# xin-fight/Research-and-Implementation-of-Image-Dehazing-Algorithm-Based-on-Vision-Transformer

Hardware: AMD Instinct MI355X
Metric: train patches/sec (128x128, embed_dim=32) (higher is better)
Workload: dtype f32; 1 GPU; Uformer_ProbSparse train step E=32 ps=128 per-GPU bs=32 fp32 Charbonnier+CR(VGG19, seeded-random weights) + AdamW (BASELINE configs[1]); global_batch=32, parallelism=dp1, arithmetic=fp32 storage/accumulate; products 6xbf16 MFMA, dropped <= 2^-24, split_terms=6

## Files before the change

### include/dehaze_hip.h

```cpp
#ifndef DEHAZE_HIP_H
#define DEHAZE_HIP_H

#include <stdint.h>

#ifdef __cplusplus
extern "C" {
#endif

#define DHZ_OK 0
#define DHZ_EINVAL (-22)
#define DHZ_ELAUNCH (-5)

#define DHZ_F32 0
#define DHZ_BF16 1

#define DHZ_NTOK 64
#define DHZ_NTOP 25

int dhz_abi_version(void);
const char* dhz_last_error(void);
const char* dhz_build_id(void);
int dhz_set_reserved_cus(int k);
int dhz_get_reserved_cus(void);
int dhz_grid_cus(void);
// ... 83 lines not shown
                        const float* bd, const float* b2, const float* drop_scale, float* out, float* xn_save, float* stats_save,
                        float* u_save, float* tp_save, float* z_save, int B, int Hres, int Wres, int C, void* stream);
int dhz_leff_prepack6(const float* w1, const float* w2, void* w6, int C, void* stream);

int dhz_linear_fwd(const float* x, int ldx, const float* w, const float* bias, float* y, int ldy, int T, int N, int K,
                   void* stream);
int dhz_linear_dgrad(const float* dy, int ldy, const float* w, float* dx, int ldx, int T, int N, int K, void* stream);
int dhz_linear_tile(int rows, int out_features);

int dhz_linear_fwd_split(const float* x, int ldx, const float* w, const float* bias, float* y, int ldy, int T, int N, int K,
                         int terms, void* stream);
int dhz_linear_dgrad_split(const float* dy, int ldy, const float* w, float* dx, int ldx, int T, int N, int K, int terms,
                           void* stream);
int dhz_linear_fwd_split6(const float* x, int ldx, const void* w_hi, const void* w_mid, const void* w_lo, const float* bias, float* y,
                          int ldy, int T, int N, int K, void* stream);
int dhz_linear_dgrad_split6(const float* dy, int ldy, const void* w_hi, const void* w_mid, const void* w_lo, float* dx, int ldx, int T,
                            int N, int K, void* stream);
int dhz_linear_fwd_split6_res(const float* x, int ldx, const void* w_hi, const void* w_mid, const void* w_lo, const float* bias,
                              const float* res, const float* scale, float* out, int ldo, int T, int N, int K, int tokens_per_image,
                              int Hres, int Wres, int shift, int windowed, void* stream);
int dhz_linear_split6_tile(int mode, int T, int N, int K);
int dhz_linear_fwd_split_res(const float* x, int ldx, const float* w, const float* bias, const float* res, const float* scale, float* out,
                             int ldo, int T, int N, int K, int tokens_per_image, int Hres, int Wres, int shift, int windowed, int terms,
                             void* stream);
int dhz_linear_dgrad_split_scaled(const float* dy, int ldy, const float* w, const float* scale, float* dx, int ldx, int T, int N, int K,
                                  int tokens_per_image, int terms, void* stream);
int dhz_linear_fwd_bf16_res(const void* x, int ldx, const void* w, const float* bias, const void* res, const float* scale, void* out, int ldo,
                            int T, int N, int K, int tokens_per_image, int Hres, int Wres, int shift, int windowed, void* stream);
int dhz_split3_planes(const float* src, int64_t n, void* hi, void* mid, void* lo, void* stream);
int dhz_split3_planes_t(const float* src, void* hi, void* mid, void* lo, const int* desc, int nmat, int ntiles, void* stream);
int dhz_bf16_transpose_batched(const float* src, void* dst, const int* desc, int nmat, int ntiles, void* stream);
int dhz_linear_wgrad_split(const float* dy, int ldy, const float* x, int ldx, int T, int nmat, int nper, int K, float* const* dw,
                           float* const* db, const float* row_scale, int rows_per_scale, int terms, void* stream);

int dhz_linear_fwd_bf16(const void* x, int ldx, const void* w, const float* bias, void* y, int ldy, int T, int N, int K,
                        void* stream);
int dhz_linear_dgrad_bf16(const void* dy, int ldy, const void* w, void* dx, int ldx, int T, int N, int K, void* stream);
int dhz_linear_wgrad_bf16(const void* dy, int ldy, const void* x, int ldx, int T, int nmat, int nper, int K,
                          float* const* dw, float* const* db, void* stream);

int dhz_gelu_fwd_dt(const void* u, void* y, int64_t n, int dtype, void* stream);
int dhz_gelu_bwd_dt(const void* dy, const void* u, void* du, int64_t n, const float* scale, int64_t elems_per_scale, int dtype, void* stream);
int dhz_ln_partition_fwd_dt(const void* x, const float* gamma, const float* beta, void* xw, float* stats, int B, int Hres,
                            int Wres, int C, int shift, int partition, int dtype, void* stream);
int dhz_ln_partition_bwd_dt(const void* dxw, const void* x, const float* gamma, const float* stats, const void* dres, void* dx,
                            float* dgamma, float* dbeta, int B, int Hres, int Wres, int C, int shift, int partition, int dtype,
                            void* stream);
int dhz_ln_partition_bwd_lay(const void* dxw, const void* x, const float* gamma, const float* stats, const void* dres, void* dx,
                             float* dgamma, float* dbeta, int B, int Hres, int Wres, int C, int shift, int partition, int dres_windowed,
                             int dx_windowed, int dx_shift, int dtype, void* stream);
int dhz_ln_partition_bwd_lay2(const void* dxw, const void* x, const float* gamma, const float* stats, const void* dres, void* dx,
                              float* dgamma, float* dbeta, int B, int Hres, int Wres, int C, int shift, int partition, int dres_windowed,
                              int dx_windowed, int dx_shift, void* dx2, const float* scale2, int dtype, void* stream);
int dhz_reverse_residual_fwd_dt(const void* yw, const void* shortcut, const float* scale, void* out, int B, int Hres, int Wres,
                                int C, int shift, int partition, int dtype, void* stream);
int dhz_reverse_residual_bwd_dt(const void* dout, const float* scale, void* dyw, int B, int Hres, int Wres, int C, int shift,
                                int partition, int dtype, void* stream);
int dhz_leff_dwconv_fwd_dt(const void* u, const float* w, const float* b, void* t, void* z, int B, int Hres, int Wres, int Ch,
                           int dtype, void* stream);
int dhz_leff_dwconv_bwd_dt(const void* dz, const void* u, const void* t, const float* w, void* du, float* dw, float* db, int B,
                           int Hres, int Wres, int Ch, int dtype, void* stream);
int dhz_leff_dwconv_bwd_scaled_dt(const void* dz, const void* u, const void* t, const float* w, void* du, float* dw, float* db,
                                  const float* dz_scale, int B, int Hres, int Wres, int Ch, int dtype, void* stream);
int dhz_leff_dwconv_bwd_dy(const float* dy, int ldy, const void* w2t_hi, const void* w2t_mid, const void* w2t_lo, const float* u,
                           const float* tpre, const float* wd, float* du, float* dw, float* db, const float* dz_scale, int B, int Hres,
                           int Wres, int C, int Ch, void* stream);
// ... 169 lines not shown
```

### research-and-implementation-of-image-dehazing-algorithm-based-on-vision-transformer_amd/dehaze_hip/_lib.py

```python
import ctypes
import os

_HERE = os.path.dirname(os.path.abspath(__file__))
LIB_PATH = os.environ.get("DHZ_LIB_PATH") or os.path.join(_HERE, "libdehaze_hip.so")

c_f = ctypes.c_void_p
c_p = ctypes.c_void_p
c_i = ctypes.c_int
c_l = ctypes.c_int64
c_fl = ctypes.c_float

SIGNATURES = {
    "dhz_abi_version": [],
    "dhz_last_error": [],
    "dhz_build_id": [],
    "dhz_set_reserved_cus": [ctypes.c_int],
    "dhz_gelu_fwd_dt": [ctypes.c_void_p, ctypes.c_void_p, ctypes.c_int64, ctypes.c_int, ctypes.c_void_p],
    "dhz_gelu_bwd_dt": [ctypes.c_void_p, ctypes.c_void_p, ctypes.c_void_p, ctypes.c_int64, ctypes.c_void_p, ctypes.c_int64, ctypes.c_int, ctypes.c_void_p],
    "dhz_get_reserved_cus": [],
    "dhz_set_deterministic": [ctypes.c_int],
    "dhz_get_deterministic": [],
    "dhz_set_det_workspace": [ctypes.c_void_p, ctypes.c_size_t],
    "dhz_grid_cus": [],
    "dhz_ps_attn_fwd": [c_f, c_f, c_f, c_i, c_p, c_f, c_f, c_f, c_i, c_p, c_i, c_i, c_i, c_i, c_p],
# ... 35 lines not shown
    "dhz_winograd43_conv3x3_pool": [c_f, c_f, c_f, c_f, c_f, c_i, c_i, c_i, c_i, c_i, c_p],
    "dhz_winograd_conv3x3_slices": [c_f, c_f, c_f, c_i, c_f, c_f, c_f, c_f, c_i, c_i, c_i, c_i, c_i, c_i, c_p],
    "dhz_winograd43_conv3x3_slices": [c_f, c_f, c_f, c_i, c_f, c_f, c_f, c_f, c_i, c_i, c_i, c_i, c_i, c_i, c_p],
    "dhz_winograd_slices": [c_i, c_i, c_i, c_i, c_i],
    "dhz_maxpool2x2_blocked_fwd": [c_f, c_f, c_i, c_i, c_i, c_p],
    "dhz_maxpool2x2_blocked_bwd": [c_f, c_f, c_f, c_i, c_i, c_i, c_p],
    "dhz_layout_blocked8": [c_f, c_f, c_i, c_i, c_i, c_i, c_f, c_i, c_p],
    "dhz_leff_fused_fwd": [c_f] * 16 + [c_i, c_i, c_i, c_i, c_p],
    "dhz_leff_fused_fwd6": [c_f] * 15 + [c_i, c_i, c_i, c_i, c_p],
    "dhz_leff_prepack6": [c_f, c_f, c_p, c_i, c_p],
    "dhz_linear_fwd": [c_f, c_i, c_f, c_f, c_f, c_i, c_i, c_i, c_i, c_p],
    "dhz_linear_dgrad": [c_f, c_i, c_f, c_f, c_i, c_i, c_i, c_i, c_p],
    "dhz_input_proj_fwd": [c_f, c_f, c_f, c_f, c_i, c_i, c_i, c_i, c_fl, c_p],
    "dhz_input_proj_bwd": [c_f, c_f, c_f, c_f, c_f, c_i, c_i, c_i, c_i, c_fl, c_p],
    "dhz_conv4s2_fwd": [c_f, c_f, c_f, c_f, c_i, c_i, c_i, c_i, c_i, c_p],
    "dhz_conv4s2_dgrad": [c_f, c_f, c_f, c_i, c_i, c_i, c_i, c_i, c_p],
    "dhz_conv4s2_wgrad": [c_f, c_f, c_f, c_f, c_i, c_i, c_i, c_i, c_i, c_p],
    "dhz_input_proj_fwd_dt": [c_f, c_f, c_f, c_f, c_i, c_i, c_i, c_i, c_fl, c_i, c_p],
    "dhz_input_proj_bwd_dt": [c_f, c_f, c_f, c_f, c_f, c_i, c_i, c_i, c_i, c_fl, c_i, c_p],
    "dhz_thin_conv3x3_fwd_dt": [c_f, c_f, c_f, c_f, c_i, c_i, c_i, c_i, c_i, c_p],
    "dhz_thin_conv3x3_dgrad_dt": [c_f, c_f, c_f, c_i, c_i, c_i, c_i, c_i, c_p],
    "dhz_thin_conv3x3_wgrad_dt": [c_f, c_f, c_f, c_f, c_i, c_i, c_i, c_i, c_i, c_p],
    "dhz_vgg_prepack_bf16": [c_f, c_f, c_i, c_i, c_i, c_p],
    "dhz_vgg_conv3x3_bf16": [c_f, c_f, c_f, c_i, c_f, c_f, c_f, c_i, c_i, c_i, c_i, c_i, c_p],
    "dhz_maxpool2x2_nhwc_bf16_fwd": [c_f, c_f, c_i, c_i, c_i, c_i, c_p],
    "dhz_maxpool2x2_nhwc_bf16_bwd": [c_f, c_f, c_f, c_i, c_i, c_i, c_i, c_p],
    "dhz_l1_pair_fwd_bf16": [c_f, c_f, c_f, c_f, c_l, c_p],
    "dhz_l1_pair_bwd_bf16": [c_f, c_f, c_f, c_f, c_f, c_l, c_p],
    "dhz_im2col_k4s2_bf16": [c_f, c_f, c_i, c_i, c_i, c_i, c_p],
    "dhz_col2im_k4s2_bf16": [c_f, c_f, c_i, c_i, c_i, c_i, c_p],
    "dhz_linear_fwd_split": [c_f, c_i, c_f, c_f, c_f, c_i, c_i, c_i, c_i, c_i, c_p],
    "dhz_linear_dgrad_split": [c_f, c_i, c_f, c_f, c_i, c_i, c_i, c_i, c_i, c_p],
    "dhz_linear_wgrad_split": [c_f, c_i, c_f, c_i, c_i, c_i, c_i, c_i, c_f, c_f, c_f, c_i, c_i, c_p],
    "dhz_linear_fwd_split6": [c_f, c_i, c_p, c_p, c_p, c_f, c_f, c_i, c_i, c_i, c_i, c_p],
    "dhz_linear_dgrad_split6": [c_f, c_i, c_p, c_p, c_p, c_f, c_i, c_i, c_i, c_i, c_p],
    "dhz_linear_fwd_split6_res": [c_f, c_i, c_p, c_p, c_p, c_f, c_f, c_f, c_f, c_i, c_i, c_i, c_i, c_i, c_i, c_i, c_i, c_i, c_p],
    "dhz_linear_fwd_split_res": [c_f, c_i, c_f, c_f, c_f, c_f, c_f, c_i, c_i, c_i, c_i, c_i, c_i, c_i, c_i, c_i, c_i, c_p],
    "dhz_linear_fwd_bf16_res": [c_f, c_i, c_f, c_f, c_f, c_f, c_f, c_i, c_i, c_i, c_i, c_i, c_i, c_i, c_i, c_i, c_p],
    "dhz_linear_dgrad_split_scaled": [c_f, c_i, c_f, c_f, c_f, c_i, c_i, c_i, c_i, c_i, c_i, c_p],
    "dhz_ln_partition_bwd_lay2": [c_f, c_f, c_f, c_f, c_f, c_f, c_f, c_f, c_i, c_i, c_i, c_i, c_i, c_i, c_i, c_i, c_i, c_f, c_f, c_i, c_p],
    "dhz_ln_partition_bwd_lay": [c_f, c_f, c_f, c_f, c_f, c_f, c_f, c_f, c_i, c_i, c_i, c_i, c_i, c_i, c_i, c_i, c_i, c_i, c_p],
    "dhz_split3_planes": [c_f, c_l, c_p, c_p, c_p, c_p],
    "dhz_split3_planes_t": [c_f, c_p, c_p, c_p, c_p, c_i, c_i, c_p],
    "dhz_linear_fwd_bf16": [c_f, c_i, c_f, c_f, c_f, c_i, c_i, c_i, c_i, c_p],
    "dhz_bf16_transpose_batched": [c_f, c_p, c_p, c_i, c_i, c_p],
    "dhz_linear_dgrad_bf16": [c_f, c_i, c_f, c_f, c_i, c_i, c_i, c_i, c_p],
    "dhz_linear_wgrad_bf16": [c_f, c_i, c_f, c_i, c_i, c_i, c_i, c_i, c_p, c_p, c_p],
    "dhz_ln_partition_fwd_dt": [c_f, c_f, c_f, c_f, c_f, c_i, c_i, c_i, c_i, c_i, c_i, c_i, c_p],
    "dhz_ln_partition_bwd_dt": [c_f, c_f, c_f, c_f, c_f, c_f, c_f, c_f, c_i, c_i, c_i, c_i, c_i, c_i, c_i, c_p],
    "dhz_reverse_residual_fwd_dt": [c_f, c_f, c_f, c_f, c_i, c_i, c_i, c_i, c_i, c_i, c_i, c_p],
    "dhz_reverse_residual_bwd_dt": [c_f, c_f, c_f, c_i, c_i, c_i, c_i, c_i, c_i, c_i, c_p],
    "dhz_leff_dwconv_fwd_dt": [c_f, c_f, c_f, c_f, c_f, c_i, c_i, c_i, c_i, c_i, c_p],
    "dhz_leff_dwconv_bwd_dt": [c_f, c_f, c_f, c_f, c_f, c_f, c_f, c_i, c_i, c_i, c_i, c_i, c_p],
    "dhz_leff_dwconv_bwd_scaled_dt": [c_f, c_f, c_f, c_f, c_f, c_f, c_f, c_f, c_i, c_i, c_i, c_i, c_i, c_p],
    "dhz_leff_dwconv_bwd_dy": [c_f, c_i, c_p, c_p, c_p, c_f, c_f, c_f, c_f, c_f, c_f, c_f, c_i, c_i, c_i, c_i, c_i, c_p],
    "dhz_ps_attn_fwd_dt": [c_f, c_f, c_f, c_i, c_p, c_f, c_f, c_f, c_i, c_p, c_i, c_i, c_i, c_i, c_i, c_p],
    "dhz_ps_attn_bwd_dt": [c_f, c_f, c_f, c_i, c_f, c_f, c_p, c_f, c_i, c_f, c_f, c_f, c_i, c_f, c_i, c_i, c_i, c_i, c_i, c_p],
    "dhz_linear_wgrad": [c_f, c_i, c_f, c_i, c_i, c_i, c_i, c_f, c_f, c_p],
    "dhz_linear_wgrad_rs": [c_f, c_i, c_f, c_i, c_i, c_i, c_i, c_f, c_f, c_f, c_i, c_p],
    "dhz_linear_wgrad_multi": [c_f, c_i, c_f, c_i, c_i, c_i, c_i, c_i, c_p, c_p, c_p],
    "dhz_ln_partition_fwd": [c_f, c_f, c_f, c_f, c_f, c_i, c_i, c_i, c_i, c_i, c_i, c_p],
    "dhz_ln_partition_bwd": [c_f, c_f, c_f, c_f, c_f, c_f, c_f, c_f, c_i, c_i, c_i, c_i, c_i, c_i, c_p],
    "dhz_reverse_residual_fwd": [c_f, c_f, c_f, c_f, c_i, c_i, c_i, c_i, c_i, c_i, c_p],
    "dhz_reverse_residual_bwd": [c_f, c_f, c_f, c_i, c_i, c_i, c_i, c_i, c_i, c_p],
    "dhz_leff_dwconv_fwd": [c_f, c_f, c_f, c_f, c_f, c_i, c_i, c_i, c_i, c_p],
    "dhz_leff_dwconv_bwd": [c_f, c_f, c_f, c_f, c_f, c_f, c_f, c_i, c_i, c_i, c_i, c_p],
# ... 80 lines not shown
```

### research-and-implementation-of-image-dehazing-algorithm-based-on-vision-transformer_amd/dehaze_hip/fused.py

```python
import torch
from torch.autograd import Function

from . import _lib, ops
from .ops import NTOK, _grad_buf, _int_array, _p, _ptr_array, _ready, _require_gpu, _stream

SUPPORTED_C = (32, 64, 128)
ENABLED = True
ATTN_FUSED_C128_MAX_HW = int(__import__("os").environ.get("DHZ_FUSED_C128_MAX_HW", "1024"))
ATTN_FUSED_BWD_C = (32,)


def _fused_bwd_widths():
    return () if ops.DETERMINISTIC else ATTN_FUSED_BWD_C
ATTN_FUSED_P6 = __import__("os").environ.get("DHZ_FUSED_P6", "1") != "0"
ATTN_FUSED_P6_C = (64, 128)
ATTN_FUSED_PAD_P6_C = (64, 128)
LEFF_FUSED = True
LEFF_FUSED_C = (32, 64)
LEFF_FUSED_C64_MAX_T = 262144
LEFF_FUSED_P6 = __import__("os").environ.get("DHZ_LEFF_P6", "1") != "0"
LEFF_FUSED_P6_C = (64,)
LEFF_BWD_DZ = __import__("os").environ.get("DHZ_LEFF_BWD_DZ", "1") != "0"
LEFF_BWD_DZ_C = (32, 64, 128)

# ... 267 lines not shown

def _attn_bwd(rec, dout, windowed=False, daw_pre=None):
    if rec.kind == "attn_fused_bwd":
        assert not windowed
        return _attn_bwd_fused(rec, dout)
    x, gamma, stats, xn, qkv, cx, rank, bias, mask, dscale, wq_, wk_, wv_, wo_ = rec.saved
    wq, bq, wk, bk, wv, bv, wo, bo, gamma_p, beta_p, table_p = rec.params
    B, Hres, Wres, C, shift, H = rec.geom
    d = C // H
    dout = dout.contiguous()
    dev = x.device
    T = B * Hres * Wres
    B_ = T // NTOK
    f32 = dict(device=dev, dtype=torch.float32)
    if daw_pre is not None:
        daw = daw_pre.view(T, C)
        dctx = ops.gemm_dgrad(daw, wo_)
        g_wo, g_bo = _wgrad(daw, 0, cx, wo, bo)
    elif windowed:
        daw = dout.view(T, C)
        rs = (dscale, Hres * Wres) if dscale is not None else None
        dctx = ops.gemm_dgrad(daw, wo_, rs)
        g_wo, g_bo = _wgrad(daw, 0, cx, wo, bo, rs)
    else:
        daw = torch.empty((T, C), device=dev, dtype=dout.dtype)
        _lib.call("dhz_reverse_residual_bwd_dt", _p(dout), _p(dscale), _p(daw), B, Hres, Wres, C, shift, 1, ops._dt(dout), _stream())
        dctx = ops.gemm_dgrad(daw, wo_)
        g_wo, g_bo = _wgrad(daw, 0, cx, wo, bo)
    dqkv = torch.empty_like(qkv)
    parts = _lib.load().dhz_ps_attn_bwd_parts_d(B_, H, d)
    dpart = torch.empty((parts, NTOK, NTOK), **f32) if bias is not None else None
    ops.ps_attn_bwd_launch(qkv, dqkv, bias, mask, rank, dctx, dpart, B_, H, d)
    dtable = _table_backward(dpart, parts, table_p, H, dev) if bias is not None else None
    dxn = ops.gemm_dgrad(dqkv, ops.cat_rows([wq_.detach(), wk_.detach(), wv_.detach()]))
    g_wq, g_bq, g_wk, g_bk, g_wv, g_bv = ops.linear_wgrad(dqkv, 0, xn, [(wq, bq), (wk, bk), (wv, bv)])
    dx, dgamma, dbeta = _ln_backward(dxn, x, gamma_p, beta_p, gamma, stats, dout, B, Hres, Wres, C, shift, 1, dres_windowed=windowed)
    return (dx, dgamma, dbeta, g_wq, g_bq, g_wk, g_bk, g_wv, g_bv, g_wo, g_bo, dtable)


def fused_c128_ok(HW):
    return HW <= ATTN_FUSED_C128_MAX_HW or not torch.is_grad_enabled()


def use_fused_attn(C, dtype, heads, HW):
    return ENABLED and dtype == torch.float32 and C == 32 * heads and (C in (32, 64) or (C == 128 and fused_c128_ok(HW)))


def takes_node(block, tensor_mask=False, pad=False):
    h = block.num_heads
    return block.attn.variant == "probsparse" and block.win_size == 8 and block.dim in (16 * h, 32 * h, 64 * h) and not tensor_mask \
        and not (pad and torch.is_grad_enabled())


class _AttnNode(Function):

    @staticmethod
    def forward(ctx, fused, x, gamma, beta, wq, bq, wk, bk, wv, bv, wo, bo, table, idx, mask, dscale, Hres, Wres, shift, H, pad, grad_mode):
        train = grad_mode and any(ctx.needs_input_grad)
        out, rec = (_attn_fused_fwd if fused else _attn_chain_fwd)(train, x, gamma, beta, wq, bq, wk, bk, wv, bv, wo, bo, table, idx, mask,
                                                                   dscale, Hres, Wres, shift, H, pad)
        if rec is not None:
            ctx.save_for_backward(*rec.saved)
            rec.saved = ()
        ctx.rec = rec
        return out

    @staticmethod
    def backward(ctx, dout):
# ... 71 lines not shown
    gwd, gbd = _grad_buf(wd), _grad_buf(bd)
    fold = dscale is not None and dout.dtype == torch.float32 and L % 32 == 0
    zscale = dscale if fold else None
    if dscale is not None and not fold:
        dy = torch.empty((T, C), device=dev, dtype=dout.dtype)
        _lib.call("dhz_reverse_residual_bwd_dt", _p(dout), _p(dscale), _p(dy), B, L, 1, C, 0, 0, ops._dt(dout), _stream())
    else:
        dy = dout.view(T, C)
    planes = None
    if LEFF_BWD_DZ and C in LEFF_BWD_DZ_C and u.dtype == torch.float32 and dy.dtype == torch.float32 and ops.SPLIT_BF16 == 6:
        planes = ops.split_planes_t(w2_ if w2_.is_contiguous() else w2_.contiguous())
        if planes is not None and any(_p(pl) % 16 for pl in planes):
            planes = None
    dz = ops.gemm_dgrad(dy, w2_) if planes is None else None
    g_w2, g_b2 = _wgrad(dy, 0, z, w2, b2, (dscale, L) if fold else None)
    du = torch.empty_like(u)

    def dwconv_bwd(pdw, pdb):
        if planes is None:
            _lib.call("dhz_leff_dwconv_bwd_scaled_dt", _p(dz), _p(u), _p(tg), _p(wdc), _p(du), pdw, pdb, _p(zscale), B, Hres, Wres, Ch,
                      ops._dt(u), _stream())
        else:
            _lib.call("dhz_leff_dwconv_bwd_dy", _p(dy), dy.stride(0), _p(planes[0]), _p(planes[1]), _p(planes[2]), _p(u), _p(tg), _p(wdc),
                      _p(du), pdw, pdb, _p(zscale), B, Hres, Wres, C, Ch, _stream())

    if gwd is not None and gbd is not None:
        dwconv_bwd(_p(gwd), _p(gbd))
        _ready(wd, bd)
        g_wd = g_bd = None
    else:
        dwb = torch.zeros((Ch * 10,), **f32)
        dwconv_bwd(dwb.data_ptr(), dwb.data_ptr() + 4 * Ch * 9)
        g_wd, g_bd = dwb[:Ch * 9].view(Ch, 1, 3, 3), dwb[Ch * 9:]
    dxn = ops.gemm_dgrad(du, w1_)
    g_w1, g_b1 = _wgrad(du, 0, xn, w1, b1)
    if dx2 is not None:
        dx, dgamma, dbeta = _ln_backward(dxn, x, gamma_p, beta_p, gamma, stats, dout, B, Hres, Wres, C, 0, 0, dx2=dx2)
    elif dx_window is None:
        dx, dgamma, dbeta = _ln_backward(dxn, x, gamma_p, beta_p, gamma, stats, dout, B, L, 1, C, 0, 0)
    else:
        dx, dgamma, dbeta = _ln_backward(dxn, x, gamma_p, beta_p, gamma, stats, dout, B, Hres, Wres, C, 0, 0, dx_window=dx_window)
    return (dx, dgamma, dbeta, g_w1, g_b1, g_wd, g_bd, g_w2, g_b2)


class _LeffBranch(Function):

    @staticmethod
    def forward(ctx, x, gamma, beta, w1, b1, wd, bd, w2, b2, dscale, Hres, Wres, grad_mode):
        train = grad_mode and any(ctx.needs_input_grad)
        out, rec = _leff_fwd(train, x, gamma, beta, w1, b1, wd, bd, w2, b2, dscale, Hres, Wres)
        if rec is not None:
            ctx.save_for_backward(*rec.saved)
            rec.saved = ()
        ctx.rec = rec
        return out

    @staticmethod
    def backward(ctx, dout):
        rec = ctx.rec
        rec.saved = ctx.saved_tensors
        g = _leff_bwd(rec, dout)
        rec.saved = ()
        return g + (None, None, None, None)


class _FfnBranch(Function):

    @staticmethod
# ... 5 lines not shown
        dev = x.device
        xn = torch.empty((T, C), device=dev, dtype=x.dtype)
        stats = torch.empty((T, 2), device=dev, dtype=torch.float32)
        _lib.call("dhz_ln_partition_fwd_dt", _p(x), _p(gamma), _p(beta), _p(xn), _p(stats), B, L, 1, C, 0, 0, ops._dt(x), _stream())
        u = ops.gemm_fwd(xn, w1, b1)
        z = torch.empty_like(u)
        _lib.call("dhz_gelu_fwd_dt", _p(u), _p(z), u.numel(), ops._dt(u), _stream())
        out = ops.gemm_fwd_res(z, w2, b2, x.view(T, C), dscale, B, L, 1, 0, False).view(B, L, C)
        if grad_mode and any(ctx.needs_input_grad):
            ctx.save_for_backward(x, gamma, stats, xn, u, z, dscale, w1, w2)
            ctx.params = (w1, b1, w2, b2, gamma, beta)
            ctx.geom = (B, L, C)
        return out

    @staticmethod
    def backward(ctx, dout):
        x, gamma, stats, xn, u, z, dscale, w1_, w2_ = ctx.saved_tensors
        w1, b1, w2, b2, gamma_p, beta_p = ctx.params
        B, L, C = ctx.geom
        T = B * L
        Ch = u.shape[1]
        dout = dout.contiguous()
        fold = dscale is not None and dout.dtype == torch.float32 and L % 32 == 0
        if dscale is not None and not fold:
            dy = torch.empty((T, C), device=x.device, dtype=dout.dtype)
            _lib.call("dhz_reverse_residual_bwd_dt", _p(dout), _p(dscale), _p(dy), B, L, 1, C, 0, 0, ops._dt(dout), _stream())
        else:
            dy = dout.view(T, C)
        dz = ops.gemm_dgrad(dy, w2_)
        g_w2, g_b2 = _wgrad(dy, 0, z, w2, b2, (dscale, L) if fold else None)
        du = torch.empty_like(u)
        _lib.call("dhz_gelu_bwd_dt", _p(dz), _p(u), _p(du), u.numel(), _p(dscale) if fold else None, L * Ch if fold else 0, ops._dt(u),
                  _stream())
        dxn = ops.gemm_dgrad(du, w1_)
        g_w1, g_b1 = _wgrad(du, 0, xn, w1, b1)
        dx, dgamma, dbeta = _ln_backward(dxn, x, gamma_p, beta_p, gamma, stats, dout, B, L, 1, C, 0, 0)
        return (dx, dgamma, dbeta, g_w1, g_b1, g_w2, g_b2, None, None)


def ffn_branch(x, norm, mlp, dscale):
    return _FfnBranch.apply(x, norm.weight, norm.bias, mlp.fc1.weight, mlp.fc1.bias, mlp.fc2.weight, mlp.fc2.bias, dscale,
                            torch.is_grad_enabled())


def leff_branch(x, norm, mlp, dscale, Hres, Wres):
    return _LeffBranch.apply(x, norm.weight, norm.bias, mlp.linear1[0].weight, mlp.linear1[0].bias,
                             mlp.dwconv[0].weight, mlp.dwconv[0].bias, mlp.linear2[0].weight, mlp.linear2[0].bias,
                             dscale, Hres, Wres, torch.is_grad_enabled())


DUAL_BF16 = True
BLOCK_NODE = True


class _BlockNode(Function):
    NA, NL = 19, 11

    @staticmethod
    def forward(ctx, fused, x, *args):
        a, l, grad_mode = args[:_BlockNode.NA], args[_BlockNode.NA:_BlockNode.NA + _BlockNode.NL], args[-1]
        train = grad_mode and any(ctx.needs_input_grad)
        x1, ra = (_attn_fused_fwd if fused else _attn_chain_fwd)(train, x, *a)
        out, rl = _leff_fwd(train, x1, *l)
        if train:
            ctx.na = len(ra.saved)
            ctx.save_for_backward(*ra.saved, *rl.saved)
            ra.saved = rl.saved = ()
        ctx.recs = (ra, rl)
# ... 30 lines not shown
```

### research-and-implementation-of-image-dehazing-algorithm-based-on-vision-transformer_amd/dehaze_hip/ops.py

```python
import collections
import ctypes

import os

import torch
from torch.autograd import Function

from . import _lib

NTOK, NTOP = 64, 25
NTOK16, NTOP16 = 16, 15
WINDOWS = {NTOK: 8, NTOK16: 4}


def _win_of(N):
    try:
        return WINDOWS[int(N)]
    except KeyError:
        raise NotImplementedError(f"windows of {N} tokens: the HIP kernels exist for 4x4 and 8x8 windows (16 or 64 tokens) only") from None

KERNEL_TIMING = None


def _stream():
# ... 645 lines not shown
            _lib.call("dhz_linear_wgrad", *lead, N, K, _p(grp[0][1]), _p(grp[0][2]), _stream())
        off += n * N


def linear_wgrad(dy, off, x, params, row_scale=None):
    T, K = x.shape
    q, tq = (64, 64) if dy.dtype == BF16 else (16, 16)
    slots, targets, inplace = [], [], []
    for w, b in params:
        pair = None
        if not w.requires_grad and (b is None or not b.requires_grad):
            dw = db = None
        elif T % tq or K % q or w.shape[0] % q:
            raise RuntimeError(f"dehaze_hip: Linear weight gradient for T={T}, N={w.shape[0]}, K={K}: the HIP kernel needs T in {tq}s "
                               f"and N, K in {q}s for {dy.dtype} (there is deliberately no library fallback)")
        else:
            pair = _grad_pair(w, b)
            dw, db = pair or (torch.zeros(w.shape, device=w.device, dtype=torch.float32),
                              torch.zeros(b.shape, device=b.device, dtype=torch.float32) if b is not None else None)
            inplace += [w, b] if pair else []
        targets.append((w.shape[0], dw, db))
        slots += [None, None] if dw is None or pair else [dw, db]
    if len(inplace) == 2 * len(params):
        _wgrad_launch(dy, off, x, targets, row_scale)
    else:
        for N, dw, db in targets:
            if dw is not None:
                _wgrad_launch(dy, off, x, [(N, dw, db)], row_scale)
            off += N
    _ready(*inplace)
    return tuple(slots)


def cat_rows(ts):
    t0 = ts[0]
    end = t0.data_ptr() + t0.numel() * t0.element_size()
    base = t0.untyped_storage().data_ptr()
    ok = t0.is_contiguous() and not t0.requires_grad
    for t in ts[1:]:
        ok = ok and t.is_contiguous() and not t.requires_grad and t.dtype == t0.dtype and t.device == t0.device \
            and t.shape[1:] == t0.shape[1:] and t.data_ptr() == end and t.untyped_storage().data_ptr() == base
        if not ok:
            break
        end += t.numel() * t.element_size()
    if not ok:
        return torch.cat(list(ts), 0)
    rows = sum(t.shape[0] for t in ts)
    shape = (rows,) + tuple(t0.shape[1:])
    return t0.as_strided(shape, t0.stride())


class _LinearTokens(Function):

    @staticmethod
    def forward(ctx, x, *wb):
        _require_gpu(x)
        params = [(wb[i], wb[i + 1]) for i in range(0, len(wb), 2)]
        if len(params) == 1:
            W, b = params[0]
        else:
            W = cat_rows([w.detach() for w, _ in params])
            b = cat_rows([b_.detach() for _, b_ in params])
        if x.dtype == BF16:
            W = bf16_copy(W)
        y = gemm_fwd(x, W, b)
        ctx.save_for_backward(x, W)
# ... 386 lines not shown
```

Baseline: 1043 patches/s.

## Fuse linear dgrad and wgrad into a single pass over dy

Adds a HIP kernel that computes dx = dy·W and dW/db = dy^T·x together for the QKV and first-MLP linears. It streams token tiles of dy and x once, splits them into bf16 planes in shared memory with double buffering, and runs 6-term MFMA for both products. Weight gradients are accumulated in registers and flushed with fp32 atomics. This saves one read and split of dy and one kernel launch per layer, at the cost of atomics (nondeterministic, disabled in deterministic mode) and a grid capped at the CU count.

Measured after the change: 1062 patches/s, median of 6. 1.9% higher.

```diff
diff --git a/include/dehaze_hip.h b/include/dehaze_hip.h
--- a/include/dehaze_hip.h
+++ b/include/dehaze_hip.h
@@ -139,6 +139,9 @@
 int dhz_bf16_transpose_batched(const float* src, void* dst, const int* desc, int nmat, int ntiles, void* stream);
 int dhz_linear_wgrad_split(const float* dy, int ldy, const float* x, int ldx, int T, int nmat, int nper, int K, float* const* dw,
                            float* const* db, const float* row_scale, int rows_per_scale, int terms, void* stream);
+int dhz_linear_bwd_pair(const float* dy, int ldy, const float* x, int ldx, const void* wt_hi, const void* wt_mid, const void* wt_lo,
+                        float* dx, int T, int nmat, int nper, int K, float* const* dw, float* const* db, void* stream);
+int dhz_linear_bwd_pair_grid(int T, int N, int K);
 
 int dhz_linear_fwd_bf16(const void* x, int ldx, const void* w, const float* bias, void* y, int ldy, int T, int N, int K,
                         void* stream);
diff --git a/research-and-implementation-of-image-dehazing-algorithm-based-on-vision-transformer_amd/csrc/linear_bwd_pair.hip b/research-and-implementation-of-image-dehazing-algorithm-based-on-vision-transformer_amd/csrc/linear_bwd_pair.hip
--- /dev/null
+++ b/research-and-implementation-of-image-dehazing-algorithm-based-on-vision-transformer_amd/csrc/linear_bwd_pair.hip
@@ -0,0 +1,292 @@
+#include <type_traits>
+#include <utility>
+#include "bf16_pipe.h"
+
+namespace {
+
+constexpr int MAXMAT = 4;
+constexpr int ST = 32;
+constexpr int NT = 512;
+constexpr int IMG = ST * 64 * 2;
+
+struct PairOut {
+    float* dw[MAXMAT];
+    float* db[MAXMAT];
+    int nper;
+};
+
+template <int N, int K>
+struct PairCfg {
+    static constexpr int NS = N / 64;
+    static constexpr int PIECE = (NS + 1) * IMG, STAGE = 3 * PIECE;
+    static constexpr int KSPLIT = 8 / (2 * (K / 16));
+    static constexpr int PART = KSPLIT == 2 ? 2 * 4 * 64 * 16 : 0;
+    static constexpr size_t SMEM = 2 * (size_t)STAGE + PART;
+    static_assert((size_t)N * K * 4 <= 2 * (size_t)STAGE && (size_t)ST * N * 4 <= 2 * (size_t)STAGE, "the epilogue reuses the stage buffers");
+};
+
+template <class F, int... I>
+__device__ __forceinline__ void static_for(std::integer_sequence<int, I...>, F&& f) { (f(std::integral_constant<int, I>{}), ...); }
+constexpr int piece_of(int gi, int ng, int np) {
+    for (int p = 0; p < np; ++p)
+        if (p * ng / np == gi) return p;
+    return -1;
+}
+
+template <int N, int K>
+__global__ __launch_bounds__(NT) void linear_bwd_pair_kernel(const float* __restrict__ dy, int ldy, const float* __restrict__ x, int ldx,
+                                                             const uint16_t* __restrict__ wt_hi, const uint16_t* __restrict__ wt_mid,
+                                                             const uint16_t* __restrict__ wt_lo, float* __restrict__ dx, int T,
+                                                             PairOut out) {
+    using C = PairCfg<N, K>;
+    constexpr int NS = C::NS, PIECE = C::PIECE, STAGE = C::STAGE, KSPLIT = C::KSPLIT;
+    constexpr int QPR = N / 4, QA = ST * QPR / NT;
+    constexpr int XE = ST * K / NT;
+    constexpr bool SAMECOL = NT % QPR == 0;
+    constexpr int NDB = SAMECOL ? 1 : QA;
+    constexpr int WB = K / 32;
+    constexpr int KS = N / 32 / KSPLIT;
+    static_assert(QA * NT == ST * QPR && (XE == 4 || XE == 2), "a stage is a whole number of quads per thread");
+    extern __shared__ __attribute__((aligned(16))) unsigned char smem[];
+    const int t = threadIdx.x, lane = t & 63, w = t >> 6;
+    const int i16 = lane & 15, g = lane >> 4;
+    const int wn = w & 3, wk = w >> 2;
+    const int tb = w & 1, cb = KSPLIT == 2 ? (w >> 1) & 1 : w >> 1, half = KSPLIT == 2 ? w >> 2 : 0;
+    const int nst = T / ST;
+    const int st0 = (int)((long long)nst * blockIdx.x / gridDim.x), st1 = (int)((long long)nst * (blockIdx.x + 1) / gridDim.x);
+
+    dhz_u32x4 wf[3][KS];
+    {
+        const uint16_t* const pl[3] = {wt_hi, wt_mid, wt_lo};
+#pragma unroll
+        for (int pc = 0; pc < 3; ++pc)
+#pragma unroll
+            for (int s = 0; s < KS; ++s)
+                wf[pc][s] = *reinterpret_cast<const dhz_u32x4*>(pl[pc] + (size_t)(16 * cb + i16) * N + 32 * (half * KS + s) + 8 * g);
+    }
+    f32x4 acc[NS][WB];
+#pragma unroll
+    for (int a = 0; a < NS; ++a)
+#pragma unroll
+        for (int b = 0; b < WB; ++b) acc[a][b] = f32x4{0.f, 0.f, 0.f, 0.f};
+    float dbacc[NDB][4];
+#pragma unroll
+    for (int i = 0; i < NDB; ++i)
+#pragma unroll
+        for (int c = 0; c < 4; ++c) dbacc[i][c] = 0.f;
+
+    f32x4 ra[QA], rx = f32x4{0.f, 0.f, 0.f, 0.f};
+    int a_off[QA];
+    unsigned pa[QA];
+#pragma unroll
+    for (int i = 0; i < QA; ++i) {
+        const int q = t + NT * i, row = q / QPR, c4 = q % QPR, ch = c4 >> 1;
+        a_off[i] = (ch >> 3) * IMG + dhz_off_tr<64>(row, ch & 7) + 8 * (c4 & 1);
+        pa[i] = (unsigned)((row * ldy + 4 * c4) * 4);
+    }
+    const int xrow = (t * XE) / K, xcol = (t * XE) % K;
+    const int x_off = NS * IMG + dhz_off_tr<64>(xrow, xcol >> 3) + 2 * (xcol & 7);
+    const unsigned px = (unsigned)((xrow * ldx + xcol) * 4);
+    auto gload = [&](int st) {
+        const size_t tok0 = (size_t)st * ST;
+        const char* const da = reinterpret_cast<const char*>(dy) + tok0 * ldy * 4;
+        const char* const xa = reinterpret_cast<const char*>(x) + tok0 * ldx * 4;
+#pragma unroll
+        for (int i = 0; i < QA; ++i) ra[i] = *reinterpret_cast<const f32x4*>(da + pa[i]);
+        if constexpr (XE == 4) rx = *reinterpret_cast<const f32x4*>(xa + px);
+        else {
+            const dhz_f32x2 v = *reinterpret_cast<const dhz_f32x2*>(xa + px);
+            rx[0] = v[0]; rx[1] = v[1];
+        }
+    };
+    typedef uint32_t u32x2 __attribute__((ext_vector_type(2)));
+    auto swrite_piece = [&](int buf, auto p_) {
+        constexpr int p = decltype(p_)::value;
+        unsigned char* const S = smem + buf * STAGE;
+        dhz_u32x4 hi, mid, lo;
+        if constexpr (p < QA) {
+            dhz_split8x3_np(ra[p], ra[p], hi, mid, lo);
+            *reinterpret_cast<u32x2*>(S + a_off[p]) = u32x2{hi[0], hi[1]};
+            *reinterpret_cast<u32x2*>(S + PIECE + a_off[p]) = u32x2{mid[0], mid[1]};
+            *reinterpret_cast<u32x2*>(S + 2 * PIECE + a_off[p]) = u32x2{lo[0], lo[1]};
+#pragma unroll
+            for (int c = 0; c < 4; ++c) dbacc[SAMECOL ? 0 : p][c] += ra[p][c];
+        } else {
+            dhz_split8x3_np(rx, rx, hi, mid, lo);
+            if constexpr (XE == 4) {
+                *reinterpret_cast<u32x2*>(S + x_off) = u32x2{hi[0], hi[1]};
+                *reinterpret_cast<u32x2*>(S + PIECE + x_off) = u32x2{mid[0], mid[1]};
+                *reinterpret_cast<u32x2*>(S + 2 * PIECE + x_off) = u32x2{lo[0], lo[1]};
+            } else {
+                *reinterpret_cast<uint32_t*>(S + x_off) = hi[0];
+                *reinterpret_cast<uint32_t*>(S + PIECE + x_off) = mid[0];
+                *reinterpret_cast<uint32_t*>(S + 2 * PIECE + x_off) = lo[0];
+            }
+        }
+    };
+    auto swrite = [&](int buf) { static_for(std::make_integer_sequence<int, QA + 1>{}, [&](auto p_) { swrite_piece(buf, p_); }); };
+    f32x4 dprev = f32x4{0.f, 0.f, 0.f, 0.f};
+    f32x4* const part = reinterpret_cast<f32x4*>(smem + 2 * STAGE);
+    auto drain = [&](int st) {
+        if (KSPLIT == 2) {
+            if (half) return;
+            dprev += part[((st & 1) * 4 + (w & 3)) * 64 + lane];
+        }
+        *reinterpret_cast<f32x4*>(dx + ((size_t)st * ST + 16 * tb + i16) * K + 16 * cb + 4 * g) = dprev;
+    };
+
+    if (st0 < st1) {
+        gload(st0);
+        swrite(st0 & 1);
+        if (st0 + 1 < st1) gload(st0 + 1);
+    }
+    __syncthreads();
+    constexpr int TA[6] = {2, 0, 1, 1, 0, 0}, TB[6] = {0, 2, 1, 0, 1, 0};
+    auto stage = [&](int st, auto more) {
+        constexpr bool MORE = decltype(more)::value;
+        const int buf = st & 1;
+        const unsigned char* const S = smem + buf * STAGE;
+        if (st > st0) drain(st - 1);
+        constexpr int NG = NS + KS;
+        dhz_s16x8 bf[3][WB], fr[2][3];
+        f32x4 dacc = f32x4{0.f, 0.f, 0.f, 0.f};
+        auto frags = [&](auto gi_, dhz_s16x8(&f)[3]) {
+            constexpr int gi = decltype(gi_)::value;
+            if constexpr (gi < NS) {
+                const int nb = wn * NS + gi;
+#pragma unroll
+                for (int pc = 0; pc < 3; ++pc) f[pc] = dhz_tr_frag<64>(S + pc * PIECE + (nb >> 2) * IMG, 8 * g, nb & 3, lane);
+            } else {
+                const int ks = half * KS + gi - NS;
+#pragma unroll
+                for (int pc = 0; pc < 3; ++pc)
+                    f[pc] = *reinterpret_cast<const dhz_s16x8*>(S + pc * PIECE + (ks >> 1) * IMG + dhz_off_tr<64>(16 * tb + i16, (ks & 1) * 4 + g));
+            }
+        };
+#pragma unroll
+        for (int pc = 0; pc < 3; ++pc)
+#pragma unroll
+            for (int b = 0; b < WB; ++b) bf[pc][b] = dhz_tr_frag<64>(S + pc * PIECE + NS * IMG, 8 * g, wk * WB + b, lane);
+        frags(std::integral_constant<int, 0>{}, fr[0]);
+        static_for(std::make_integer_sequence<int, NG>{}, [&](auto gi_) {
+            constexpr int gi = decltype(gi_)::value;
+            constexpr int NM = gi < NS ? 6 * WB : 6;
+            if constexpr (gi + 1 < NG) frags(std::integral_constant<int, gi + 1>{}, fr[(gi + 1) & 1]);
+            __builtin_amdgcn_sched_barrier(0);
+            if constexpr (gi < NS) {
+#pragma unroll
+                for (int term = 0; term < 6; ++term)
+#pragma unroll
+                    for (int b = 0; b < WB; ++b) acc[gi][b] = dhz_mfma_bf16(fr[gi & 1][TA[term]], bf[TB[term]][b], acc[gi][b]);
+            } else {
+#pragma unroll
+                for (int term = 0; term < 6; ++term)
+                    dacc = dhz_mfma_bf16(__builtin_bit_cast(dhz_s16x8, wf[TB[term]][gi - NS]), fr[gi & 1][TA[term]], dacc);
+            }
+            constexpr int p = piece_of(gi, NG, QA + 1);
+            if constexpr (MORE && p >= 0) swrite_piece(buf ^ 1, std::integral_constant<int, p>{});
+#pragma unroll
+            for (int i = 0; i < NM; ++i) {
+                __builtin_amdgcn_sched_group_barrier(0x008, 1, 0);
+                __builtin_amdgcn_sched_group_barrier(0x202, 3, 0);
+            }
+            __builtin_amdgcn_sched_barrier(0);
+        });
+        if (KSPLIT == 2 && half) part[(buf * 4 + (w & 3)) * 64 + lane] = dacc;
+        else dprev = dacc;
+        if (st + 2 < st1) gload(st + 2);
+        asm volatile("s_waitcnt lgkmcnt(0)" ::: "memory");
+        __builtin_amdgcn_s_barrier();
+        asm volatile("" ::: "memory");
+    };
+    for (int st = st0; st + 1 < st1; ++st) stage(st, std::true_type{});
+    if (st0 < st1) stage(st1 - 1, std::false_type{});
+    if (st0 < st1) drain(st1 - 1);
+    float* const Cs = reinterpret_cast<float*>(smem);
+#pragma unroll
+    for (int a = 0; a < NS; ++a)
+#pragma unroll
+        for (int b = 0; b < WB; ++b)
+#pragma unroll
+            for (int j = 0; j < 4; ++j) Cs[((wn * NS + a) * 16 + 4 * g + j) * K + (wk * WB + b) * 16 + i16] = acc[a][b][j];
+    __syncthreads();
+    for (int e = t; e < N * K; e += NT) {
+        const int n = e / K, mat = n / out.nper;
+        atomicAdd(out.dw[mat] + (size_t)(n - mat * out.nper) * K + e % K, Cs[e]);
+    }
+    bool do_db = false;
+#pragma unroll
+    for (int m = 0; m < MAXMAT; ++m) do_db = do_db || out.db[m] != nullptr;
+    if (do_db) {
+        __syncthreads();
+        float* const red = reinterpret_cast<float*>(smem);
+        constexpr int ROWS = SAMECOL ? NT / QPR : ST;
+#pragma unroll
+        for (int i = 0; i < NDB; ++i) {
+            const int q = t + NT * i;
+            *reinterpret_cast<f32x4*>(red + (q / QPR) * N + 4 * (q % QPR)) = f32x4{dbacc[i][0], dbacc[i][1], dbacc[i][2], dbacc[i][3]};
+        }
+        __syncthreads();
+        if (t < N) {
+            float tot = 0.f;
+            for (int r = 0; r < ROWS; ++r) tot += red[r * N + t];
+            const int mat = t / out.nper;
+            if (out.db[mat]) atomicAdd(out.db[mat] + t - mat * out.nper, tot);
+        }
+    }
+}
+
+int pair_grid(int T) {
+    const int nst = T / ST, cus = dhz_num_cus();
+    return cus < nst ? cus : nst;
+}
+
+bool pair_shape(int N, int K) { return (N == 128 && K == 32) || (N == 256 && K == 64) || (N == 192 && K == 64); }
+
+template <int N, int K>
+void launch(int grid, hipStream_t s, const float* dy, int ldy, const float* x, int ldx, const uint16_t* hi, const uint16_t* mid,
+            const uint16_t* lo, float* dx, int T, const PairOut& out) {
+    constexpr size_t smem = PairCfg<N, K>::SMEM;
+    dhz_allow_smem(&linear_bwd_pair_kernel<N, K>, smem);
+    hipLaunchKernelGGL((linear_bwd_pair_kernel<N, K>), dim3(grid), dim3(NT), smem, s, dy, ldy, x, ldx, hi, mid, lo, dx, T, out);
+}
+
+}
+
+extern "C" int dhz_linear_bwd_pair_grid(int T, int N, int K) {
+    if (T <= 0 || T % ST || !pair_shape(N, K)) return 0;
+    return pair_grid(T);
+}
+
+extern "C" int dhz_linear_bwd_pair(const float* dy, int ldy, const float* x, int ldx, const void* wt_hi, const void* wt_mid,
+                                   const void* wt_lo, float* dx, int T, int nmat, int nper, int K, float* const* dw, float* const* db,
+                                   void* stream) {
+    const char* who = "dhz_linear_bwd_pair";
+    DHZ_REQUIRE(!dhz_det(), "%s: accumulates with fp32 atomics: not available in deterministic mode (run dhz_linear_fwd_split6 on the "
+                            "planes of W^T and dhz_linear_wgrad_split)", who);
+    DHZ_REQUIRE(dy && x && wt_hi && wt_mid && wt_lo && dx && dw, "%s: null pointer", who);
+    DHZ_REQUIRE(nmat >= 1 && nmat <= MAXMAT, "%s: nmat=%d must be 1..%d", who, nmat, MAXMAT);
+    DHZ_REQUIRE(T > 0 && T % ST == 0, "%s: T=%d must be a positive multiple of %d", who, T, ST);
+    DHZ_REQUIRE(nper > 0 && nper % 16 == 0 && pair_shape(nmat * nper, K),
+                "%s: N=%d (nmat=%d x nper=%d) K=%d: instances are N x K = 128 x 32, 256 x 64 and 192 x 64", who, nmat * nper, nmat, nper, K);
+    const int N = nmat * nper;
+    DHZ_REQUIRE(ldy % 4 == 0 && ldy >= N, "%s: ldy=%d must be a multiple of 4 and at least N=%d", who, ldy, N);
+    DHZ_REQUIRE(ldx % 4 == 0 && ldx >= K, "%s: ldx=%d must be a multiple of 4 and at least K=%d", who, ldx, K);
+    DHZ_REQUIRE(!(((uintptr_t)dy | (uintptr_t)x | (uintptr_t)wt_hi | (uintptr_t)wt_mid | (uintptr_t)wt_lo | (uintptr_t)dx) & 15),
+                "%s: dy, x, the planes and dx must be 16-byte aligned", who);
+    PairOut out = {};
+    for (int i = 0; i < nmat; ++i) {
+        DHZ_REQUIRE(dw[i], "%s: null dw[%d]", who, i);
+        out.dw[i] = dw[i];
+        out.db[i] = db ? db[i] : nullptr;
+    }
+    out.nper = nper;
+    const int grid = pair_grid(T);
+    hipStream_t s = (hipStream_t)stream;
+    const uint16_t *hi = (const uint16_t*)wt_hi, *mid = (const uint16_t*)wt_mid, *lo = (const uint16_t*)wt_lo;
+    if (N == 128) launch<128, 32>(grid, s, dy, ldy, x, ldx, hi, mid, lo, dx, T, out);
+    else if (N == 256) launch<256, 64>(grid, s, dy, ldy, x, ldx, hi, mid, lo, dx, T, out);
+    else launch<192, 64>(grid, s, dy, ldy, x, ldx, hi, mid, lo, dx, T, out);
+    DHZ_CHECK_LAUNCH(who);
+    return DHZ_OK;
+}
diff --git a/research-and-implementation-of-image-dehazing-algorithm-based-on-vision-transformer_amd/dehaze_hip/_lib.py b/research-and-implementation-of-image-dehazing-algorithm-based-on-vision-transformer_amd/dehaze_hip/_lib.py
--- a/research-and-implementation-of-image-dehazing-algorithm-based-on-vision-transformer_amd/dehaze_hip/_lib.py
+++ b/research-and-implementation-of-image-dehazing-algorithm-based-on-vision-transformer_amd/dehaze_hip/_lib.py
@@ -91,6 +91,8 @@
     "dhz_linear_fwd_split": [c_f, c_i, c_f, c_f, c_f, c_i, c_i, c_i, c_i, c_i, c_p],
     "dhz_linear_dgrad_split": [c_f, c_i, c_f, c_f, c_i, c_i, c_i, c_i, c_i, c_p],
     "dhz_linear_wgrad_split": [c_f, c_i, c_f, c_i, c_i, c_i, c_i, c_i, c_f, c_f, c_f, c_i, c_i, c_p],
+    "dhz_linear_bwd_pair": [c_f, c_i, c_f, c_i, c_p, c_p, c_p, c_f, c_i, c_i, c_i, c_i, c_f, c_f, c_p],
+    "dhz_linear_bwd_pair_grid": [c_i, c_i, c_i],
     "dhz_linear_fwd_split6": [c_f, c_i, c_p, c_p, c_p, c_f, c_f, c_i, c_i, c_i, c_i, c_p],
     "dhz_linear_dgrad_split6": [c_f, c_i, c_p, c_p, c_p, c_f, c_i, c_i, c_i, c_i, c_p],
     "dhz_linear_fwd_split6_res": [c_f, c_i, c_p, c_p, c_p, c_f, c_f, c_f, c_f, c_i, c_i, c_i, c_i, c_i, c_i, c_i, c_i, c_i, c_p],
diff --git a/research-and-implementation-of-image-dehazing-algorithm-based-on-vision-transformer_amd/dehaze_hip/fused.py b/research-and-implementation-of-image-dehazing-algorithm-based-on-vision-transformer_amd/dehaze_hip/fused.py
--- a/research-and-implementation-of-image-dehazing-algorithm-based-on-vision-transformer_amd/dehaze_hip/fused.py
+++ b/research-and-implementation-of-image-dehazing-algorithm-based-on-vision-transformer_amd/dehaze_hip/fused.py
@@ -323,8 +323,8 @@
     dpart = torch.empty((parts, NTOK, NTOK), **f32) if bias is not None else None
     ops.ps_attn_bwd_launch(qkv, dqkv, bias, mask, rank, dctx, dpart, B_, H, d)
     dtable = _table_backward(dpart, parts, table_p, H, dev) if bias is not None else None
-    dxn = ops.gemm_dgrad(dqkv, ops.cat_rows([wq_.detach(), wk_.detach(), wv_.detach()]))
-    g_wq, g_bq, g_wk, g_bk, g_wv, g_bv = ops.linear_wgrad(dqkv, 0, xn, [(wq, bq), (wk, bk), (wv, bv)])
+    dxn, (g_wq, g_bq, g_wk, g_bk, g_wv, g_bv) = ops.linear_bwd_pair(dqkv, xn, ops.cat_rows([wq_.detach(), wk_.detach(), wv_.detach()]),
+                                                                    [(wq, bq), (wk, bk), (wv, bv)])
     dx, dgamma, dbeta = _ln_backward(dxn, x, gamma_p, beta_p, gamma, stats, dout, B, Hres, Wres, C, shift, 1, dres_windowed=windowed)
     return (dx, dgamma, dbeta, g_wq, g_bq, g_wk, g_bk, g_wv, g_bv, g_wo, g_bo, dtable)
 
@@ -462,8 +462,7 @@
         dwb = torch.zeros((Ch * 10,), **f32)
         dwconv_bwd(dwb.data_ptr(), dwb.data_ptr() + 4 * Ch * 9)
         g_wd, g_bd = dwb[:Ch * 9].view(Ch, 1, 3, 3), dwb[Ch * 9:]
-    dxn = ops.gemm_dgrad(du, w1_)
-    g_w1, g_b1 = _wgrad(du, 0, xn, w1, b1)
+    dxn, (g_w1, g_b1) = ops.linear_bwd_pair(du, xn, w1_, [(w1, b1)])
     if dx2 is not None:
         dx, dgamma, dbeta = _ln_backward(dxn, x, gamma_p, beta_p, gamma, stats, dout, B, Hres, Wres, C, 0, 0, dx2=dx2)
     elif dx_window is None:
@@ -535,8 +534,7 @@
         du = torch.empty_like(u)
         _lib.call("dhz_gelu_bwd_dt", _p(dz), _p(u), _p(du), u.numel(), _p(dscale) if fold else None, L * Ch if fold else 0, ops._dt(u),
                   _stream())
-        dxn = ops.gemm_dgrad(du, w1_)
-        g_w1, g_b1 = _wgrad(du, 0, xn, w1, b1)
+        dxn, (g_w1, g_b1) = ops.linear_bwd_pair(du, xn, w1_, [(w1, b1)])
         dx, dgamma, dbeta = _ln_backward(dxn, x, gamma_p, beta_p, gamma, stats, dout, B, L, 1, C, 0, 0)
         return (dx, dgamma, dbeta, g_w1, g_b1, g_w2, g_b2, None, None)
 
diff --git a/research-and-implementation-of-image-dehazing-algorithm-based-on-vision-transformer_amd/dehaze_hip/ops.py b/research-and-implementation-of-image-dehazing-algorithm-based-on-vision-transformer_amd/dehaze_hip/ops.py
--- a/research-and-implementation-of-image-dehazing-algorithm-based-on-vision-transformer_amd/dehaze_hip/ops.py
+++ b/research-and-implementation-of-image-dehazing-algorithm-based-on-vision-transformer_amd/dehaze_hip/ops.py
@@ -701,6 +701,43 @@
     return tuple(slots)
 
 
+LINEAR_BWD_PAIR = os.environ.get("DHZ_LINEAR_BWD_PAIR", "1") != "0"
+LINEAR_BWD_PAIR_BUILT = ((128, 32), (256, 64), (192, 64))
+LINEAR_BWD_PAIR_SHAPES = ((128, 32), (256, 64), (192, 64))
+
+
+def _bwd_pair_operands(dy, x, W, params):
+    T, K = x.shape
+    N = W.shape[0]
+    if not LINEAR_BWD_PAIR or (N, K) not in LINEAR_BWD_PAIR_SHAPES or DETERMINISTIC or SPLIT_BF16 != 6 or T % 32:
+        return None
+    if dy.dtype != torch.float32 or x.dtype != torch.float32 or dy.stride(1) != 1 or x.stride(1) != 1 or dy.stride(0) % 4 or x.stride(0) % 4:
+        return None
+    if _p(dy) % 16 or _p(x) % 16 or len({w.shape[0] for w, _ in params}) != 1 or sum(w.shape[0] for w, _ in params) != N:
+        return None
+    if any(not w.requires_grad or (b is not None and not b.requires_grad) for w, b in params):
+        return None
+    planes = split_planes_t(W)
+    if planes is None or any(_p(pl) % 16 for pl in planes):
+        return None
+    pairs = [_grad_pair(w, b) for w, b in params]
+    return (planes, pairs) if all(pr is not None for pr in pairs) else None
+
+
+def linear_bwd_pair(dy, x, W, params):
+    W = W if W.is_contiguous() else W.contiguous()
+    took = _bwd_pair_operands(dy, x, W, params)
+    if took is None:
+        return gemm_dgrad(dy, W), linear_wgrad(dy, 0, x, params)
+    planes, pairs = took
+    T, K = x.shape
+    dx = torch.empty((T, K), device=dy.device, dtype=dy.dtype)
+    _lib.call("dhz_linear_bwd_pair", _p(dy), dy.stride(0), _p(x), x.stride(0), *[_p(pl) for pl in planes], _p(dx), T, len(params),
+              params[0][0].shape[0], K, _ptr_array([_p(gw) for gw, _ in pairs]), _ptr_array([_p(gb) for _, gb in pairs]), _stream())
+    _ready(*[p for wb in params for p in wb])
+    return dx, (None,) * (2 * len(params))
+
+
 def cat_rows(ts):
     t0 = ts[0]
     end = t0.data_ptr() + t0.numel() * t0.element_size()
```
